# alanqrwang/nwhead

Hardware: AMD Instinct MI355X
Metric: query-predictions/sec (higher is better)
Workload: dtype f32; 1 GPU; K3 predict('full'): B=256 queries/step vs bank N=50000 d=512 C=200, bank sharded 1-way, 26 query batches coalesced per launch; B=256, N_support=50000, d=512, C=200, parallelism=support-shard x1

## Files before the change

### nwhead_amd/csrc/fused.hip

```cpp
#include <mutex>
#include <utility>
#include <vector>
#include "fused_impl.h"

namespace nw {

#define NW_EXTERN_FUSED_KIND(K) extern template int launch_fused_kind<K>(const FusedArgs&, const FusedPlan&);
NW_FOR_EACH_KIND(NW_EXTERN_FUSED_KIND)
#undef NW_EXTERN_FUSED_KIND

namespace {
struct TileTimer {
    bool on = false;
    std::vector<std::pair<hipEvent_t, hipEvent_t>> ev;
    std::vector<std::pair<hipEvent_t, hipEvent_t>> pool;
    std::mutex mu;
} g_tt;
}

int tile_timer_start(hipStream_t st) {
    if (!g_tt.on) return -1;
    std::lock_guard<std::mutex> lk(g_tt.mu);
    std::pair<hipEvent_t, hipEvent_t> p;
    if (!g_tt.pool.empty()) {
        p = g_tt.pool.back();
        g_tt.pool.pop_back();
    } else if (hipEventCreate(&p.first) != hipSuccess || hipEventCreate(&p.second) != hipSuccess) {
        return -1;
    }
    (void)hipEventRecord(p.first, st);
    g_tt.ev.push_back(p);
    return (int)g_tt.ev.size() - 1;
}
void tile_timer_stop(int slot, hipStream_t st) {
    if (slot < 0) return;
    std::lock_guard<std::mutex> lk(g_tt.mu);
    if (slot < (int)g_tt.ev.size()) (void)hipEventRecord(g_tt.ev[slot].second, st);
}
int tile_timer_enable(bool on) {
    std::lock_guard<std::mutex> lk(g_tt.mu);
    g_tt.on = on;
    return NW_OK;
}
int tile_timer_read(double* total_us, int64_t* launches) {
    std::lock_guard<std::mutex> lk(g_tt.mu);
    double tot = 0;
    for (auto& p : g_tt.ev) {
        float ms = 0.f;
        if (hipEventSynchronize(p.second) != hipSuccess || hipEventElapsedTime(&ms, p.first, p.second) != hipSuccess)
            return NW_ERR_LAUNCH;
        tot += (double)ms * 1e3;
        g_tt.pool.push_back(p);
    }
    if (total_us) *total_us = tot;
    if (launches) *launches = (int64_t)g_tt.ev.size();
    g_tt.ev.clear();
    return NW_OK;
}

namespace {
int device_cu_count() {
    static int n = [] {
        int dev = 0, v = 0;
        if (hipGetDevice(&dev) != hipSuccess) return 256;
        if (hipDeviceGetAttribute(&v, hipDeviceAttributeMultiprocessorCount, dev) != hipSuccess || v <= 0) return 256;
        return v;
    }();
    return n;
}
bool env_flag(int k) { return knob(k) == 1; }
}

inline size_t al256(size_t x) { return (x + 255) & ~(size_t)255; }

size_t fused_layout(int64_t B, int64_t n_stiles, int BS, char* base, FusedWs* ws, int64_t C) {
    size_t off = 0;
    auto take = [&](size_t bytes) {
        char* p = base ? base + off : nullptr;
        off += al256(bytes);
        return p;
    };
    FusedWs w;
    w.m = reinterpret_cast<float*>(take((size_t)n_stiles * B * 4));
    w.den = reinterpret_cast<float*>(take((size_t)n_stiles * B * 4));
    w.nrun = reinterpret_cast<int*>(take((size_t)n_stiles * 4));
    w.lab = reinterpret_cast<int*>(take((size_t)n_stiles * BS * 4));
    w.num = reinterpret_cast<float*>(take((size_t)n_stiles * BS * B * 4));
    w.runid = reinterpret_cast<int*>(take(((size_t)n_stiles * BS + 64) * 4));
    w.bnd = reinterpret_cast<int*>(take((size_t)n_stiles * 2 * 4));
    w.ctab = reinterpret_cast<int*>(take((size_t)C * (3 + 4) * 4));
    if (ws) *ws = w;
    return off;
}

namespace {

constexpr int MTHREADS = 512, MENT = 4, MTPT = 16;
template <bool PARTIAL, int MQ, int TMODE>
__global__ __launch_bounds__(MTHREADS) void nw_merge_runs_kernel(
    const float* __restrict__ ws_m, const float* __restrict__ ws_den, const int* __restrict__ ws_nrun,
    const int* __restrict__ ws_lab, const float* __restrict__ ws_num, float* __restrict__ out,
    float* __restrict__ lse, float* __restrict__ m_out, float* __restrict__ den_out,
    float* __restrict__ num_out, int B, int C, int n_stiles, int BS, const int* __restrict__ ctab) {
    constexpr bool TABLES = TMODE != 0;
    constexpr bool LTAB = TMODE == 1;
    constexpr int ML = MTHREADS / MQ;
    constexpr int MNS = MQ + 1;
    constexpr int NW = MTHREADS / 64;
    constexpr float LN2 = 0.693147180559945309417f;
    static_assert(MQ <= 32 && (MQ & (MQ - 1)) == 0, "a wave holds whole groups of MQ queries");
    extern __shared__ __attribute__((aligned(16))) char smem[];
    float* red = reinterpret_cast<float*>(smem);
    float* Ms = red + 2 * NW * MQ;
    float* inv_s = Ms + MQ;
    int* lds_tab = reinterpret_cast<int*>(inv_s + MQ);
    int* cnt = TMODE == 2 ? const_cast<int*>(ctab) : lds_tab;
    int* tlo = cnt + C;
    int* thi = tlo + C;
    int* ent = thi + C;
    float* res = reinterpret_cast<float*>(lds_tab + (size_t)C * (3 + MENT));
    const int tid = threadIdx.x, bq = tid & (MQ - 1), sl = tid / MQ, wave = tid >> 6;
    const int b0 = blockIdx.x * MQ;
    const int b = min(b0 + bq, B - 1);

    const bool in_regs = n_stiles <= ML * MTPT;
    float mr[MTPT], dr[MTPT];
    float M = -INFINITY;
    if (in_regs) {
#pragma unroll
        for (int u = 0; u < MTPT; ++u) {
            const int t = sl + u * ML;
            const bool ok = t < n_stiles;
            mr[u] = ok ? ws_m[(size_t)t * B + b] : -INFINITY;
            dr[u] = ok ? ws_den[(size_t)t * B + b] : 0.f;
        }
    }
    int tnr = 0, tl3[3] = {-1, -1, -1};
    const bool one_pass_tables = LTAB && n_stiles <= MTHREADS;
    if (one_pass_tables && tid < n_stiles) {
        tnr = ws_nrun[tid];
        const int* lt = ws_lab + (size_t)tid * BS;
        tl3[0] = lt[0];
        tl3[1] = lt[1];
        tl3[2] = lt[2];
    }
    if (LTAB) {
        for (int c = tid; c < C; c += MTHREADS) {
            cnt[c] = 0;
            tlo[c] = 0x7fffffff;
            thi[c] = -1;
        }
    }
    if (in_regs) {
#pragma unroll
        for (int u = 0; u < MTPT; ++u) M = fmaxf(M, mr[u]);
    } else {
        for (int t = sl; t < n_stiles; t += ML) M = fmaxf(M, ws_m[(size_t)t * B + b]);
    }
#pragma unroll
    for (int o = 32; o >= MQ; o >>= 1) M = fmaxf(M, __shfl_xor(M, o));
    if ((tid & 63) < MQ) red[wave * MQ + bq] = M;
    __syncthreads();
    if (LTAB) {
        auto add_tile = [&](int t, int nr, const int (&l3)[3]) {
            const int* lt = ws_lab + (size_t)t * BS;
            for (int r = 0; r < nr; ++r) {
                const int y = r < 3 ? l3[r] : lt[r];
                if (y < 0) continue;
                atomicMin(&tlo[y], t);
                atomicMax(&thi[y], t);
                const int slot = atomicAdd(&cnt[y], 1);
                if (slot < MENT) ent[y * MENT + slot] = t * BS + r;
            }
        };
        if (one_pass_tables) {
            if (tid < n_stiles) add_tile(tid, tnr, tl3);
        } else {
            for (int t = tid; t < n_stiles; t += MTHREADS) {
                const int* lt = ws_lab + (size_t)t * BS;
                const int l3[3] = {lt[0], lt[1], lt[2]};
                add_tile(t, ws_nrun[t], l3);
            }
        }
    }
    M = red[bq];
#pragma unroll
    for (int k = 1; k < NW; ++k) M = fmaxf(M, red[k * MQ + bq]);
    float den = 0.f;
    if (in_regs) {
#pragma unroll
        for (int u = 0; u < MTPT; ++u) den += dr[u] * __builtin_amdgcn_exp2f(mr[u] - M);
    } else {
        for (int t = sl; t < n_stiles; t += ML)
            den += ws_den[(size_t)t * B + b] * __builtin_amdgcn_exp2f(ws_m[(size_t)t * B + b] - M);
    }
#pragma unroll
    for (int o = 32; o >= MQ; o >>= 1) den += __shfl_xor(den, o);
    if ((tid & 63) < MQ) red[NW * MQ + wave * MQ + bq] = den;
    if (sl == 0) Ms[bq] = M;
    __syncthreads();
    if (LTAB) {
        for (int c = tid; c < C; c += MTHREADS) {
            const int n = cnt[c];
            if (n > 1 && n <= MENT) {
                int e[MENT];
#pragma unroll
                for (int k = 0; k < MENT; ++k) e[k] = k < n ? ent[c * MENT + k] : 0x7fffffff;
#pragma unroll
                for (int i = 1; i < MENT; ++i)
#pragma unroll
                    for (int j = MENT - 1; j >= i; --j)
                        if (e[j] < e[j - 1]) { const int x = e[j]; e[j] = e[j - 1]; e[j - 1] = x; }
#pragma unroll
                for (int k = 0; k < MENT; ++k)
                    if (k < n) ent[c * MENT + k] = e[k];
            }
        }
    }
    den = red[NW * MQ + bq];
#pragma unroll
    for (int k = 1; k < NW; ++k) den += red[NW * MQ + k * MQ + bq];
    if (sl == 0) inv_s[bq] = 1.f / den;
    const int nq = min(MQ, B - b0);
    if (sl == 0 && bq < nq) {
        if (PARTIAL) {
            m_out[b] = M * LN2;
            den_out[b] = den;
        } else if (lse) {
            lse[b] = M * LN2 + logf(den);
        }
    }
    __syncthreads();
    int P = 1;
    while (P < 64 && 2 * P * C * MQ <= MTHREADS) P <<= 1;
    for (int xx = tid; xx < C * MQ * P; xx += MTHREADS) {
        const int x = xx / P, sub = xx - x * P;
        const int c = x / MQ, q = x - c * MQ;
        const int bb = min(b0 + q, B - 1);
        const float Mq = Ms[q];
        float acc = 0.f;
        const int n = TABLES ? cnt[c] : MENT + 1;
        if (n <= MENT) {
            int e[MENT];
            float v[MENT], mt[MENT];
#pragma unroll
            for (int k = 0; k < MENT; ++k) e[k] = ent[c * MENT + (k < n ? k : 0)];
#pragma unroll
            for (int k = 0; k < MENT; ++k) {
                if (k < n) {
                    v[k] = ws_num[(size_t)e[k] * B + bb];
                    mt[k] = ws_m[(size_t)(e[k] / BS) * B + bb];
                }
            }
#pragma unroll
            for (int k = 0; k < MENT; ++k)
                if (k < n) acc += v[k] * __builtin_amdgcn_exp2f(mt[k] - Mq);
        } else {
            const int t0 = TABLES ? tlo[c] : 0, t1 = TABLES ? thi[c] : n_stiles - 1;
            for (int t = t0 + sub; t <= t1; t += P) {
                const int nr = ws_nrun[t];
                const float f = __builtin_amdgcn_exp2f(ws_m[(size_t)t * B + bb] - Mq);
                const int* lt = ws_lab + (size_t)t * BS;
                for (int r = 0; r < nr; ++r)
                    if (lt[r] == c) acc += ws_num[((size_t)t * BS + r) * B + bb] * f;
            }
        }
        if (P > 1) {
            if (n <= MENT && sub != 0) acc = 0.f;
            for (int o = P >> 1; o > 0; o >>= 1) acc += __shfl_xor(acc, o);
            if (sub != 0) continue;
        }
        if (LTAB && MQ > 1) {
            res[c * MNS + q] = acc;
        } else if (q < nq) {
            if (PARTIAL) num_out[(size_t)bb * C + c] = acc;
            else out[(size_t)bb * C + c] = logf(acc * inv_s[q] + NW_LOG_EPS);
        }
    }
    if (!LTAB || MQ == 1) return;
    __syncthreads();
    for (int x = tid; x < nq * C; x += MTHREADS) {
        const int qq = x / C, c = x - qq * C;
        if (PARTIAL) num_out[(size_t)(b0 + qq) * C + c] = res[c * MNS + qq];
        else out[(size_t)(b0 + qq) * C + c] = logf(res[c * MNS + qq] * inv_s[qq] + NW_LOG_EPS);
    }
}

__global__ __launch_bounds__(1024) void nw_class_tables_kernel(const int* __restrict__ ws_nrun, const int* __restrict__ ws_lab,
                                                                int n_stiles, int BS, int C, int* __restrict__ ctab) {
    int* cnt = ctab;
    int* tlo = cnt + C;
    int* thi = tlo + C;
    int* ent = thi + C;
    const int tid = threadIdx.x;
    for (int c = tid; c < C; c += 1024) {
        cnt[c] = 0;
        tlo[c] = 0x7fffffff;
        thi[c] = -1;
    }
    __threadfence();
    __syncthreads();
    for (int t = tid; t < n_stiles; t += 1024) {
        const int nr = ws_nrun[t];
        const int* lt = ws_lab + (size_t)t * BS;
        for (int r = 0; r < nr; ++r) {
            const int y = lt[r];
            if (y < 0) continue;
            atomicMin(&tlo[y], t);
            atomicMax(&thi[y], t);
            const int slot = atomicAdd(&cnt[y], 1);
            if (slot < MENT) ent[y * MENT + slot] = t * BS + r;
        }
    }
    __threadfence();
    __syncthreads();
    for (int c = tid; c < C; c += 1024) {
        const int n = cnt[c];
        if (n > 1 && n <= MENT) {
            int e[MENT];
#pragma unroll
            for (int k = 0; k < MENT; ++k) e[k] = k < n ? ent[c * MENT + k] : 0x7fffffff;
#pragma unroll
            for (int i = 1; i < MENT; ++i)
#pragma unroll
                for (int j = MENT - 1; j >= i; --j)
                    if (e[j] < e[j - 1]) { const int x = e[j]; e[j] = e[j - 1]; e[j - 1] = x; }
#pragma unroll
            for (int k = 0; k < MENT; ++k)
                if (k < n) ent[c * MENT + k] = e[k];
        }
    }
}

__global__ __launch_bounds__(64) void nw_run_tables_kernel(const int64_t* __restrict__ sy, int N, int C, int BS,
                                                           int* __restrict__ runid, int* __restrict__ nrun,
                                                           int* __restrict__ lab_out, int* __restrict__ bnd) {
    const int st = blockIdx.x, lane = threadIdx.x, s0 = st * BS;
    if (lane < 2) bnd[2 * st + lane] = BS;
    __syncthreads();
    int lab[3], flag[3];
#pragma unroll
    for (int u = 0; u < 3; ++u) {
        const int t = 3 * lane + u, j = s0 + t;
        int64_t y = -1;
        if (t < BS && j < N) y = sy[j];
        lab[u] = ((uint64_t)y < (uint64_t)C) ? (int)y : -1;
    }
    const int prev_last = __shfl_up(lab[2], 1);
    flag[0] = (lane == 0) || (lab[0] != prev_last);
    flag[1] = lab[1] != lab[0];
    flag[2] = lab[2] != lab[1];
    int incl = flag[0] + flag[1] + flag[2];
#pragma unroll
    for (int o = 1; o < 64; o <<= 1) {
        const int v = __shfl_up(incl, o);
        if (lane >= o) incl += v;
    }
    int id = incl - (flag[0] + flag[1] + flag[2]) - 1;
#pragma unroll
    for (int u = 0; u < 3; ++u) {
        const int t = 3 * lane + u;
        id += flag[u];
        if (t < BS) {
            runid[(size_t)s0 + t] = id;
            if (flag[u]) lab_out[(size_t)s0 + id] = lab[u];
            if (flag[u] && (id == 1 || id == 2)) bnd[2 * st + id - 1] = t;
            if (t == BS - 1) nrun[st] = id + 1;
        }
    }
}

int env_rs() {
    const int v = knob(KNOB_TILE_RS);
    return v == KNOB_UNSET ? 0 : v;
}

}

int query_area_of_workspace(void* workspace, size_t workspace_bytes, int64_t B, int64_t N, int64_t d, int64_t C, float** rows,
                            float** scale, float** norm2) {
    const size_t total = nw_fwd_workspace_bytes(B, N, d, C);
    if (!workspace || workspace_bytes < total) return NW_ERR_WORKSPACE;
    const size_t a = al256((size_t)B * (size_t)d * sizeof(float)), b = al256((size_t)B * sizeof(float));
    char* base = static_cast<char*>(workspace) + (total - a - 3 * b);
    *rows = reinterpret_cast<float*>(base);
    *scale = reinterpret_cast<float*>(base + a);
    *norm2 = reinterpret_cast<float*>(base + a + b);
    return NW_OK;
}

int launch_run_tables(const FusedWs& ws, const int64_t* sy, int N, int C, int n_stiles, int BS, hipStream_t st) {
    if (BS > 192) return NW_ERR_UNSUPPORTED;
    hipLaunchKernelGGL(nw_run_tables_kernel, dim3(n_stiles), dim3(64), 0, st, sy, N, C, BS, ws.runid, ws.nrun, ws.lab, ws.bnd);
    NW_CHECK_LAUNCH();
    return NW_OK;
}

constexpr int BANK_BS = 128;

size_t bank_tables_layout(int64_t n_stiles, char* base, FusedWs* ws) {
    size_t off = 0;
    auto take = [&](size_t bytes) {
        char* p = base ? base + off : nullptr;
        off += al256(bytes);
        return p;
    };
    int* nrun = reinterpret_cast<int*>(take((size_t)n_stiles * 4));
    int* lab = reinterpret_cast<int*>(take((size_t)n_stiles * BANK_BS * 4));
    int* runid = reinterpret_cast<int*>(take(((size_t)n_stiles * BANK_BS + 64) * 4));
    int* bnd = reinterpret_cast<int*>(take((size_t)n_stiles * 2 * 4));
    if (ws) {
        ws->nrun = nrun;
        ws->lab = lab;
        ws->runid = runid;
        ws->bnd = bnd;
    }
    return off;
}

bool bank_tables_take(const int64_t* sy, int N, int C, int n_stiles, int BS, FusedWs* ws) {
    (void)C;
    const FwdOpts& o = fwd_opts();
    if (!o.tables || BS != BANK_BS) return false;
    if (o.tables_sy != sy || o.tables_N != (int64_t)N) return false;
    if (o.tables_bytes < bank_tables_layout(n_stiles, nullptr, nullptr)) return false;
    bank_tables_layout(n_stiles, const_cast<char*>(o.tables), ws);
    return true;
}

int launch_merge_runs(const FusedWs& ws, float* out, float* lse, float* m, float* den, float* num,
                      int B, int C, int n_stiles, int BS, hipStream_t st) {
    auto lds_bytes = [&](int mq, bool tables) {
        return ((size_t)2 * (MTHREADS / 64) * mq + 2 * mq + (tables ? (size_t)C * (3 + MENT + mq + 1) : 0)) * sizeof(float);
    };
    const size_t cap = 150 * 1024;
    int mq = 1;
    const int force_mq = knob(KNOB_MERGE_MQ) == KNOB_UNSET ? 0 : knob(KNOB_MERGE_MQ);
    if (force_mq == 1 || force_mq == 16 || force_mq == 32) {
        mq = force_mq;
        if (lds_bytes(mq, true) > cap) mq = 1;
    } else if (B >= 512 && !env_flag(KNOB_MERGE_PER_QUERY)) {
        mq = n_stiles >= 128 ? 16 : 32;
        if (lds_bytes(mq, true) > cap) mq = 16;
        if (lds_bytes(mq, true) > cap) mq = 1;
    }
    const bool tables = lds_bytes(mq, true) <= cap;
    const size_t lds = lds_bytes(mq, tables);
    const int grid = (B + mq - 1) / mq;
#define NW_MERGE(P_, Q_, T_)                                                                                       \
    hipLaunchKernelGGL((nw_merge_runs_kernel<P_, Q_, T_>), dim3(grid), dim3(MTHREADS), lds, st, ws.m, ws.den, ws.nrun, \
                       ws.lab, ws.num, out, lse, m, den, num, B, C, n_stiles, BS, ws.ctab)
    if (!tables) {
        if (ws.ctab && !env_flag(KNOB_MERGE_NO_GLOBAL_TABLES)) {
            hipLaunchKernelGGL(nw_class_tables_kernel, dim3(1), dim3(1024), 0, st, ws.nrun, ws.lab, n_stiles, BS, C, ws.ctab);
            if (out) NW_MERGE(false, 1, 2); else NW_MERGE(true, 1, 2);
        } else {
            if (out) NW_MERGE(false, 1, 0); else NW_MERGE(true, 1, 0);
        }
    } else if (mq == 1) {
        if (out) NW_MERGE(false, 1, 1); else NW_MERGE(true, 1, 1);
    } else if (mq == 16) {
        if (out) NW_MERGE(false, 16, 1); else NW_MERGE(true, 16, 1);
    } else {
        if (out) NW_MERGE(false, 32, 1); else NW_MERGE(true, 32, 1);
    }
#undef NW_MERGE
    NW_CHECK_LAUNCH();
    return NW_OK;
}

int pick_rs(int64_t B, int64_t N, int64_t d, bool f16) {
    const int forced = env_rs();
    if (forced == 2 || forced == 4 || forced == 5 || forced == 6 || forced == 8 || forced == 10 || forced == 12)
        return forced;
    const int64_t nq = (B + BQ - 1) / BQ;
    if (forced == 0 && !f16 && d % BK == 0 && nq * ((N + 79) / 80) >= 480) return 5;
    if (forced == 0 && f16 && d % BK == 0 && nq * ((N + 127) / 128) >= 4 * 256) return 8;
    const int cand[] = {2, 4, 6, 8, 10, 12};
    const int ncand = f16 ? 5 : 6;
    double best = 1e30;
    int best_rs = 8;
    for (int ci = 0; ci < ncand; ++ci) {
        const int rs = cand[ci];
        const int64_t ns = (N + 16 * rs - 1) / (16 * rs);
        const int64_t nwg = nq * ns;
        const int64_t rounds = (nwg + 255) / 256;
        double cost = (double)rounds * (rs + 1.5);
        if (nwg >= 384) cost *= 0.85;
        if (cost < best - 1e-9) {
            best = cost;
            best_rs = rs;
        }
    }
    return best_rs;
}

bool half_form_shape_ok(int64_t d) {
    return d % 64 == 0 && d >= 192 && d <= (1 << 20);
}

namespace {
struct TileLds {
    size_t reg, dma;
    size_t p64, p64x2, p128;
};
template <int RS>
constexpr TileLds tile_lds() {
    if constexpr (RS > 5)
        return {FUSED_HDR + TileCfg<RS>::STAGE_BYTES, FUSED_HDR + DmaCfg<RS>::STAGE_BYTES, PCfg<RS, 1, false>::LDS_BYTES,
                PCfg<RS, 1, true>::LDS_BYTES, PCfg<RS, 2, false>::LDS_BYTES};
    else
        return {FUSED_HDR + TileCfg<RS>::STAGE_BYTES, FUSED_HDR + DmaCfg<RS>::STAGE_BYTES, 0, 0, 0};
}
TileLds tile_lds_of(int rs) {
    return rs == 2 ? tile_lds<2>() : rs == 4 ? tile_lds<4>() : rs == 5 ? tile_lds<5>() : rs == 6 ? tile_lds<6>()
         : rs == 8 ? tile_lds<8>() : rs == 10 ? tile_lds<10>() : tile_lds<12>();
}
}

FusedPlan plan_tiles(int64_t B, int64_t N, int64_t d, int form) {
    FusedPlan p = {};
    p.form = form;
    p.rs = form == FORM_HALF ? BANK_BS / 16 : pick_rs(B, N, d, form == FORM_SPLIT);
    p.BS = 16 * p.rs;
    const int64_t n_stiles = (N + p.BS - 1) / p.BS, n_qtiles = (B + BQ - 1) / BQ;
    const int64_t grid = (n_stiles + 7) / 8 * 8 * n_qtiles;
    if (grid > 0x7fffffff) p.status = NW_ERR_UNSUPPORTED;
    else p.n_stiles = (int)n_stiles, p.n_qtiles = (int)n_qtiles, p.grid = (int)grid;
    return p;
}

FusedPlan plan_fused(int64_t B, int64_t N, int64_t d, int64_t C, int form, int out, int k, bool norms, bool dot, int cus,
                     const FwdOpts& opts) {
    (void)C; (void)k;
    if (B < 0 || N < 0 || d < 0 || B >= (1 << 30) || N >= (1 << 30) || d >= (1 << 30)) {
        FusedPlan none = {};
        return none.status = NW_ERR_UNSUPPORTED, none;
    }
    FusedPlan p = plan_tiles(B, N, d, form);
    if (p.status != NW_OK) return p;
    auto refuse = [&p](int status) { p.status = status; return p; };
    if (cus <= 0) cus = device_cu_count();
    const TileLds lds = tile_lds_of(p.rs);
    const bool split = form == FORM_SPLIT;
    p.out = out;
    p.dma = (d % BK) == 0 && (uint64_t)(BQ + p.BS) * 2 * d * 4 < 0xffffffffull;
    if (form == FORM_HALF) {
        if (out != OUT_NONE || !half_form_shape_ok(d)) return refuse(NW_ERR_UNSUPPORTED);
        p.persistent = true;
    } else {
        if (!p.dma && (p.rs & 1)) return refuse(NW_ERR_UNSUPPORTED);
        p.persistent = split && out == OUT_NONE && p.rs > 5 && (p.rs == 8 || env_flag(KNOB_PERSISTENT_ANY_RS)) &&
                       p.grid >= 4 * (int64_t)cus && d >= 3 * BK && !env_flag(KNOB_NO_PERSISTENT);
    }
    p.run_tables = p.persistent;
    if (p.run_tables && p.BS > 192) return refuse(NW_ERR_UNSUPPORTED);
    if (split && (!p.dma || !norms)) return refuse(NW_ERR_INVALID_ARG);
    if (out == OUT_CAND && !split) return refuse(NW_ERR_INVALID_ARG);
    if (out == OUT_CAND && p.rs == 12) return refuse(NW_ERR_UNSUPPORTED);
    if (p.persistent) {
        p.mode = MODE_F16;
        p.split_queries = true;
        int wgs = cus & ~7;
        const int wg_cap = opts.persistent_wgs & ~7;
        if (wg_cap >= 8 && wg_cap < wgs) wgs = wg_cap;
        int variant = form == FORM_HALF ? 3 : knob(KNOB_PVAR);
        if (variant < 0 || variant > 3) {
            const double rows64 = 1.15 * ((B + 63) / 64 * 64);
            variant = (p.rs == 8 && (B + 255) / 256 * 256 <= rows64) ? 3 : ((B + 127) / 128 * 128 <= rows64) ? 2 : 1;
        }
        if (variant == 3 && p.rs != 8) variant = 2;
        if (variant == 2 && lds.p128 > 160 * 1024) variant = 0;
        if (variant == 1 && lds.p64x2 > 80 * 1024) variant = 0;
        p.variant = variant;
        p.workgroups = variant == 1 ? 2 * wgs : wgs;
        const int qg = (knob(KNOB_QG) >= 1 && knob(KNOB_QG) <= 64) ? knob(KNOB_QG) : 8;
        p.qgroup = variant != 3 ? qg : qg >= 2 ? qg / 2 : 1;
        p.lds_bytes = variant == 3 ? (size_t)P12::LDS_BYTES : variant == 2 ? lds.p128 : variant == 1 ? lds.p64x2 : lds.p64;
        return p;
    }
    if (split) {
        const int force_split = knob(KNOB_SPLIT_QUERIES) == KNOB_UNSET ? -1 : knob(KNOB_SPLIT_QUERIES);
        const bool raw_ok = force_split == 0 || (force_split < 0 && 2 * (int64_t)p.grid <= 3 * (int64_t)cus);
        p.split_queries = !raw_ok;
        p.mode = raw_ok ? MODE_F16Q : MODE_F16;
    } else {
        p.mode = !p.dma ? MODE_REG : (norms && !dot) ? MODE_DMA_SN : MODE_DMA;
    }
    p.lds_bytes = p.mode == MODE_REG ? lds.reg : lds.dma;
    return p;
}

size_t fused_workspace_bytes(int64_t B, int64_t N, int64_t d, int64_t C) {
    size_t need = 0;
    for (int form : {FORM_F32, FORM_SPLIT, FORM_HALF}) {
        if (form == FORM_HALF && !half_form_shape_ok(d)) continue;
        const int BS = plan_tiles(B, N, d, form).BS;
        const size_t n = fused_layout(B, (N + BS - 1) / BS, BS, nullptr, nullptr, C);
        need = n > need ? n : need;
    }
    return need;
}

bool fused_eligible(const float* q, const float* s, int64_t B, int64_t N, int64_t d, int64_t C) {
    const bool aligned = ((reinterpret_cast<uintptr_t>(q) | reinterpret_cast<uintptr_t>(s)) & 15) == 0;
    return N > 25 && d >= 4 && (d % 4) == 0 && aligned && B < (1 << 30) && N < (1 << 30) &&
           d < (1 << 30) && C < (1 << 30) && (8 + C) * 4 <= 160 * 1024;
}

int launch_fused(const FusedArgs& a, int form, int kind) {
    const int out = a.cand ? OUT_CAND : a.scores ? OUT_SCORES : OUT_NONE;
    const FusedPlan p = plan_fused(a.B, a.N, a.d, a.C, form, out, a.cand ? a.cand->k : 0, a.s_norm2 != nullptr,
                                   kind == NW_SCORE_DOT, 0, fwd_opts());
#define NW_KIND_CASE(K) case K: return launch_fused_kind<K>(a, p);
    switch (kind) {
        NW_FOR_EACH_KIND(NW_KIND_CASE)
        default: return NW_ERR_UNSUPPORTED;
    }
#undef NW_KIND_CASE
}

namespace {
struct KnnWs {
    CandOut cand;
    int64_t n_stiles;
    int kcp;
};
bool knn_shape_ok(int64_t B, int64_t N, int64_t d, int64_t k) {
    return B >= 0 && N > 25 && d >= BK && d % BK == 0 && k >= 1 && k <= 32 && k <= N && B < (1 << 30) && N < (1 << 30) &&
           d <= (1 << 20);
}
size_t knn_layout(int64_t B, int64_t N, int64_t d, int64_t k, int BS, char* base, KnnWs* out) {
    KnnWs w;
    w.n_stiles = (N + BS - 1) / BS;
    w.kcp = cand_slots((int)k, BS);
    size_t off = 0;
    auto take = [&](size_t bytes) {
        char* p = base ? base + off : nullptr;
        off += al256(bytes);
        return p;
    };
    const size_t slots = (size_t)B * (size_t)w.n_stiles * (size_t)w.kcp;
    w.cand.key = reinterpret_cast<unsigned*>(take(slots * 4));
    w.cand.row = reinterpret_cast<int*>(take(slots * 4));
    w.cand.q_rows = reinterpret_cast<float*>(take((size_t)B * (size_t)d * 4));
    w.cand.q_scale = reinterpret_cast<float*>(take((size_t)B * 4));
    w.cand.q_norm2 = reinterpret_cast<float*>(take((size_t)B * 4));
    w.cand.k = (int)k;
    if (out) *out = w;
    return off;
}
}

size_t knn_workspace_bytes(int64_t B, int64_t N, int64_t d, int64_t k) {
    if (!knn_shape_ok(B, N, d, k) || B == 0) return 0;
    if (pick_rs(B, N, d, true) > 10) return 0;
    size_t need = knn_layout(B, N, d, k, 16 * pick_rs(B, N, d, true), nullptr, nullptr);
    const int64_t nq = (B + BQ - 1) / BQ;
    for (int64_t qt = 1; qt <= nq && qt < 1024; ++qt) {
        const int64_t Bq = qt * BQ < B ? qt * BQ : B;
        for (int64_t n = 17; n <= N && qt * ((n + 127) / 128) < 1024; n += 16) {
            const int64_t nn = n > 26 ? n : 26;
            if (nn > N || k > nn) continue;
            const size_t x = knn_layout(Bq, nn, d, k, 16 * pick_rs(Bq, nn, d, true), nullptr, nullptr);
            need = x > need ? x : need;
        }
    }
    return need;
}

int launch_knn(const float* q, const float* s_split, const float* s_scale, const float* s_norm2, int64_t* idx, float* vals,
               void* workspace, size_t workspace_bytes, int64_t B, int64_t N, int64_t d, int64_t k, int kind, const float* ls,
               hipStream_t st) {
    if (!knn_shape_ok(B, N, d, k)) return NW_ERR_UNSUPPORTED;
    if (B == 0) return NW_OK;
    KnnWs w;
    const size_t need = knn_layout(B, N, d, k, plan_tiles(B, N, d, FORM_SPLIT).BS, static_cast<char*>(workspace), &w);
    if (!workspace || workspace_bytes < need) return NW_ERR_WORKSPACE;
    if (w.n_stiles * w.kcp >= (1ll << 31)) return NW_ERR_UNSUPPORTED;
    FusedArgs a = {};
    a.q = q, a.s = s_split, a.s_norm2 = s_norm2, a.s_scale = s_scale, a.ls = ls;
    a.B = (int)B, a.N = (int)N, a.d = (int)d, a.C = 1, a.st = st, a.cand = &w.cand;
    const int rc = launch_fused(a, FORM_SPLIT, kind);
    if (rc != NW_OK) return rc;
    return launch_topk_candidates(w.cand.key, w.cand.row, idx, vals, B, w.n_stiles * w.kcp, k, st);
}

}

extern "C" size_t nw_bank_tables_bytes(int64_t N) {
    if (N <= 0 || N > 0x7fffffffLL) return 0;
    return nw::bank_tables_layout((N + nw::BANK_BS - 1) / nw::BANK_BS, nullptr, nullptr);
}

extern "C" int nw_bank_tables_build(const int64_t* sy, int64_t N, int64_t C, void* tables, size_t tables_bytes,
                                    void* stream) {
    using namespace nw;
    if (N < 0 || C < 0 || N > 0x7fffffffLL || C > 0x7fffffffLL) return NW_ERR_INVALID_ARG;
    if (N == 0) return NW_OK;
    if (!sy || !tables || (reinterpret_cast<uintptr_t>(tables) & 15)) return NW_ERR_INVALID_ARG;
    const int64_t n_stiles = (N + BANK_BS - 1) / BANK_BS;
    FusedWs ws;
    if (tables_bytes < bank_tables_layout(n_stiles, static_cast<char*>(tables), &ws)) return NW_ERR_WORKSPACE;
    return launch_run_tables(ws, sy, (int)N, (int)C, (int)n_stiles, BANK_BS, static_cast<hipStream_t>(stream));
}
```

Baseline: 7.781 million query-predictions/s.

## Merge two query groups per merge block and batch fast-path class gathers

When the merge kernel runs with 16 queries per block, it can now launch 1024-thread blocks covering two query groups. This shares the per-block class-table build across twice as many queries and halves the grid. The class-entry path is split into a batched pass that issues several items' gathers before doing the exp/accumulate, to hide global load latency. It also packs tile/row indices to avoid a division, and walks the final output loop incrementally instead of dividing each iteration. In exchange it adds register pressure and more LDS per block, and the packing assumes BS is at most 256.

```diff
diff --git a/nwhead_amd/csrc/fused.hip b/nwhead_amd/csrc/fused.hip
--- a/nwhead_amd/csrc/fused.hip
+++ b/nwhead_amd/csrc/fused.hip
@@ -96,31 +96,38 @@
 namespace {
 
 constexpr int MTHREADS = 512, MENT = 4, MTPT = 16;
-template <bool PARTIAL, int MQ, int TMODE>
-__global__ __launch_bounds__(MTHREADS) void nw_merge_runs_kernel(
+__device__ __forceinline__ int ment_pack(int t, int r) { return (t << 8) | r; }
+template <bool PARTIAL, int MQ, int TMODE, int G>
+__global__ __launch_bounds__(MTHREADS * G) void nw_merge_runs_kernel(
     const float* __restrict__ ws_m, const float* __restrict__ ws_den, const int* __restrict__ ws_nrun,
     const int* __restrict__ ws_lab, const float* __restrict__ ws_num, float* __restrict__ out,
     float* __restrict__ lse, float* __restrict__ m_out, float* __restrict__ den_out,
     float* __restrict__ num_out, int B, int C, int n_stiles, int BS, const int* __restrict__ ctab) {
     constexpr bool TABLES = TMODE != 0;
     constexpr bool LTAB = TMODE == 1;
+    constexpr int NT = MTHREADS * G;
+    constexpr int QW = MQ * G;
     constexpr int ML = MTHREADS / MQ;
-    constexpr int MNS = MQ + 1;
-    constexpr int NW = MTHREADS / 64;
+    constexpr int MNS = QW + 1;
+    constexpr int NW = NT / 64;
+    constexpr int MITEMS = G == 2 ? 7 : MQ == 1 ? 2 : 4;
     constexpr float LN2 = 0.693147180559945309417f;
     static_assert(MQ <= 32 && (MQ & (MQ - 1)) == 0, "a wave holds whole groups of MQ queries");
+    static_assert(G == 1 || (G == 2 && QW <= 32), "two groups: one more tile-lane bit comes from the wave number");
     extern __shared__ __attribute__((aligned(16))) char smem[];
     float* red = reinterpret_cast<float*>(smem);
-    float* Ms = red + 2 * NW * MQ;
-    float* inv_s = Ms + MQ;
-    int* lds_tab = reinterpret_cast<int*>(inv_s + MQ);
+    float* Ms = red + 2 * NW * QW;
+    float* inv_s = Ms + QW;
+    int* lds_tab = reinterpret_cast<int*>(inv_s + QW);
     int* cnt = TMODE == 2 ? const_cast<int*>(ctab) : lds_tab;
     int* tlo = cnt + C;
     int* thi = tlo + C;
     int* ent = thi + C;
     float* res = reinterpret_cast<float*>(lds_tab + (size_t)C * (3 + MENT));
-    const int tid = threadIdx.x, bq = tid & (MQ - 1), sl = tid / MQ, wave = tid >> 6;
-    const int b0 = blockIdx.x * MQ;
+    const int tid = threadIdx.x, wave = tid >> 6;
+    const int bq = tid & (QW - 1);
+    const int sl = G == 1 ? tid / MQ : (wave >> 1) * (64 / MQ) + 2 * ((tid & 63) / QW) + (wave & 1);
+    const int b0 = blockIdx.x * QW;
     const int b = min(b0 + bq, B - 1);
 
     const bool in_regs = n_stiles <= ML * MTPT;
@@ -136,7 +143,7 @@
         }
     }
     int tnr = 0, tl3[3] = {-1, -1, -1};
-    const bool one_pass_tables = LTAB && n_stiles <= MTHREADS;
+    const bool one_pass_tables = LTAB && n_stiles <= NT;
     if (one_pass_tables && tid < n_stiles) {
         tnr = ws_nrun[tid];
         const int* lt = ws_lab + (size_t)tid * BS;
@@ -145,7 +152,7 @@
         tl3[2] = lt[2];
     }
     if (LTAB) {
-        for (int c = tid; c < C; c += MTHREADS) {
+        for (int c = tid; c < C; c += NT) {
             cnt[c] = 0;
             tlo[c] = 0x7fffffff;
             thi[c] = -1;
@@ -158,8 +165,8 @@
         for (int t = sl; t < n_stiles; t += ML) M = fmaxf(M, ws_m[(size_t)t * B + b]);
     }
 #pragma unroll
-    for (int o = 32; o >= MQ; o >>= 1) M = fmaxf(M, __shfl_xor(M, o));
-    if ((tid & 63) < MQ) red[wave * MQ + bq] = M;
+    for (int o = 32; o >= QW; o >>= 1) M = fmaxf(M, __shfl_xor(M, o));
+    if ((tid & 63) < QW) red[wave * QW + bq] = M;
     __syncthreads();
     if (LTAB) {
         auto add_tile = [&](int t, int nr, const int (&l3)[3]) {
@@ -170,13 +177,13 @@
                 atomicMin(&tlo[y], t);
                 atomicMax(&thi[y], t);
                 const int slot = atomicAdd(&cnt[y], 1);
-                if (slot < MENT) ent[y * MENT + slot] = t * BS + r;
+                if (slot < MENT) ent[y * MENT + slot] = ment_pack(t, r);
             }
         };
         if (one_pass_tables) {
             if (tid < n_stiles) add_tile(tid, tnr, tl3);
         } else {
-            for (int t = tid; t < n_stiles; t += MTHREADS) {
+            for (int t = tid; t < n_stiles; t += NT) {
                 const int* lt = ws_lab + (size_t)t * BS;
                 const int l3[3] = {lt[0], lt[1], lt[2]};
                 add_tile(t, ws_nrun[t], l3);
@@ -185,7 +192,7 @@
     }
     M = red[bq];
 #pragma unroll
-    for (int k = 1; k < NW; ++k) M = fmaxf(M, red[k * MQ + bq]);
+    for (int k = 1; k < NW; ++k) M = fmaxf(M, red[k * QW + bq]);
     float den = 0.f;
     if (in_regs) {
 #pragma unroll
@@ -195,12 +202,12 @@
             den += ws_den[(size_t)t * B + b] * __builtin_amdgcn_exp2f(ws_m[(size_t)t * B + b] - M);
     }
 #pragma unroll
-    for (int o = 32; o >= MQ; o >>= 1) den += __shfl_xor(den, o);
-    if ((tid & 63) < MQ) red[NW * MQ + wave * MQ + bq] = den;
+    for (int o = 32; o >= QW; o >>= 1) den += __shfl_xor(den, o);
+    if ((tid & 63) < QW) red[NW * QW + wave * QW + bq] = den;
     if (sl == 0) Ms[bq] = M;
     __syncthreads();
     if (LTAB) {
-        for (int c = tid; c < C; c += MTHREADS) {
+        for (int c = tid; c < C; c += NT) {
             const int n = cnt[c];
             if (n > 1 && n <= MENT) {
                 int e[MENT];
@@ -217,11 +224,18 @@
             }
         }
     }
-    den = red[NW * MQ + bq];
-#pragma unroll
-    for (int k = 1; k < NW; ++k) den += red[NW * MQ + k * MQ + bq];
+    const float* dred = red + NW * QW;
+    if (G == 1) {
+        den = dred[bq];
+#pragma unroll
+        for (int k = 1; k < NW; ++k) den += dred[k * QW + bq];
+    } else {
+        den = dred[bq] + dred[QW + bq];
+#pragma unroll
+        for (int k = 1; k < NW / 2; ++k) den += dred[2 * k * QW + bq] + dred[(2 * k + 1) * QW + bq];
+    }
     if (sl == 0) inv_s[bq] = 1.f / den;
-    const int nq = min(MQ, B - b0);
+    const int nq = min(QW, B - b0);
     if (sl == 0 && bq < nq) {
         if (PARTIAL) {
             m_out[b] = M * LN2;
@@ -231,58 +245,91 @@
         }
     }
     __syncthreads();
-    int P = 1;
-    while (P < 64 && 2 * P * C * MQ <= MTHREADS) P <<= 1;
-    for (int xx = tid; xx < C * MQ * P; xx += MTHREADS) {
-        const int x = xx / P, sub = xx - x * P;
-        const int c = x / MQ, q = x - c * MQ;
+    int P = 1, lgP = 0;
+    while (P < 64 && 2 * P * C * MQ <= MTHREADS) { P <<= 1; ++lgP; }
+    const int n_items = P == 1 ? C * QW : NT;
+    auto item = [&](int xx, int& c, int& q, int& sub) {
+        if (P == 1) {
+            c = xx / QW, q = xx - c * QW, sub = 0;
+            return xx < n_items;
+        }
+        const int grp = xx / MTHREADS, xg = xx - grp * MTHREADS, x = xg >> lgP;
+        c = x / MQ, q = grp * MQ + (x - c * MQ), sub = xg - (x << lgP);
+        return xg < C * MQ * P;
+    };
+    auto emit = [&](int c, int q, float acc) {
+        if (LTAB && MQ > 1) {
+            res[c * MNS + q] = acc;
+        } else if (q < nq) {
+            const int bb = b0 + q;
+            if (PARTIAL) num_out[(size_t)bb * C + c] = acc;
+            else out[(size_t)bb * C + c] = logf(acc * inv_s[q] + NW_LOG_EPS);
+        }
+    };
+    if (TABLES) {
+        for (int base = tid; base < n_items; base += NT * MITEMS) {
+            float v[MITEMS][MENT], mt[MITEMS][MENT];
+            auto fast_item = [&](int i, int& c, int& q) {
+                int sub;
+                const bool ok = base + i * NT < n_items && item(base + i * NT, c, q, sub) && sub == 0;
+                const int n = ok ? cnt[c] : MENT + 1;
+                if (n <= MENT) return n;
+                c = 0, q = 0;
+                return -1;
+            };
+#pragma unroll
+            for (int i = 0; i < MITEMS; ++i) {
+                int c, q;
+                const int n = fast_item(i, c, q);
+                const int bb = min(b0 + q, B - 1), cc = n > 0 ? c : 0;
+#pragma unroll
+                for (int k = 0; k < MENT; ++k) {
+                    const int ek = ent[cc * MENT + (k < n ? k : 0)], e = n > 0 ? ek : 0;
+                    const unsigned t = (unsigned)e >> 8, row = t * BS + (e & 255);
+                    v[i][k] = ws_num[(size_t)row * (unsigned)B + bb];
+                    mt[i][k] = ws_m[(size_t)t * (unsigned)B + bb];
+                }
+            }
+#pragma unroll
+            for (int i = 0; i < MITEMS; ++i) {
+                int c, q;
+                const int n = fast_item(i, c, q);
+                const float Mq = Ms[q];
+                float acc = 0.f;
+#pragma unroll
+                for (int k = 0; k < MENT; ++k)
+                    if (k < n) acc += v[i][k] * __builtin_amdgcn_exp2f(mt[i][k] - Mq);
+                if (n >= 0) emit(c, q, acc);
+            }
+        }
+    }
+    for (int xx = tid; xx < n_items; xx += NT) {
+        int c, q, sub;
+        if (!item(xx, c, q, sub)) continue;
+        if (TABLES && cnt[c] <= MENT) continue;
         const int bb = min(b0 + q, B - 1);
         const float Mq = Ms[q];
         float acc = 0.f;
-        const int n = TABLES ? cnt[c] : MENT + 1;
-        if (n <= MENT) {
-            int e[MENT];
-            float v[MENT], mt[MENT];
-#pragma unroll
-            for (int k = 0; k < MENT; ++k) e[k] = ent[c * MENT + (k < n ? k : 0)];
-#pragma unroll
-            for (int k = 0; k < MENT; ++k) {
-                if (k < n) {
-                    v[k] = ws_num[(size_t)e[k] * B + bb];
-                    mt[k] = ws_m[(size_t)(e[k] / BS) * B + bb];
-                }
-            }
-#pragma unroll
-            for (int k = 0; k < MENT; ++k)
-                if (k < n) acc += v[k] * __builtin_amdgcn_exp2f(mt[k] - Mq);
-        } else {
-            const int t0 = TABLES ? tlo[c] : 0, t1 = TABLES ? thi[c] : n_stiles - 1;
-            for (int t = t0 + sub; t <= t1; t += P) {
-                const int nr = ws_nrun[t];
-                const float f = __builtin_amdgcn_exp2f(ws_m[(size_t)t * B + bb] - Mq);
-                const int* lt = ws_lab + (size_t)t * BS;
-                for (int r = 0; r < nr; ++r)
-                    if (lt[r] == c) acc += ws_num[((size_t)t * BS + r) * B + bb] * f;
-            }
-        }
-        if (P > 1) {
-            if (n <= MENT && sub != 0) acc = 0.f;
-            for (int o = P >> 1; o > 0; o >>= 1) acc += __shfl_xor(acc, o);
-            if (sub != 0) continue;
-        }
-        if (LTAB && MQ > 1) {
-            res[c * MNS + q] = acc;
-        } else if (q < nq) {
-            if (PARTIAL) num_out[(size_t)bb * C + c] = acc;
-            else out[(size_t)bb * C + c] = logf(acc * inv_s[q] + NW_LOG_EPS);
-        }
+        const int t0 = TABLES ? tlo[c] : 0, t1 = TABLES ? thi[c] : n_stiles - 1;
+        for (int t = t0 + sub; t <= t1; t += P) {
+            const int nr = ws_nrun[t];
+            const float f = __builtin_amdgcn_exp2f(ws_m[(size_t)t * B + bb] - Mq);
+            const int* lt = ws_lab + (size_t)t * BS;
+            for (int r = 0; r < nr; ++r)
+                if (lt[r] == c) acc += ws_num[((size_t)t * BS + r) * B + bb] * f;
+        }
+        for (int o = P >> 1; o > 0; o >>= 1) acc += __shfl_xor(acc, o);
+        if (sub == 0) emit(c, q, acc);
     }
     if (!LTAB || MQ == 1) return;
     __syncthreads();
-    for (int x = tid; x < nq * C; x += MTHREADS) {
-        const int qq = x / C, c = x - qq * C;
+    const int dq = NT / C, dc = NT - dq * C;
+    int qq = tid / C, c = tid - qq * C;
+    for (int x = tid; x < nq * C; x += NT) {
         if (PARTIAL) num_out[(size_t)(b0 + qq) * C + c] = res[c * MNS + qq];
         else out[(size_t)(b0 + qq) * C + c] = logf(res[c * MNS + qq] * inv_s[qq] + NW_LOG_EPS);
+        qq += dq, c += dc;
+        if (c >= C) c -= C, ++qq;
     }
 }
 
@@ -309,7 +356,7 @@
             atomicMin(&tlo[y], t);
             atomicMax(&thi[y], t);
             const int slot = atomicAdd(&cnt[y], 1);
-            if (slot < MENT) ent[y * MENT + slot] = t * BS + r;
+            if (slot < MENT) ent[y * MENT + slot] = ment_pack(t, r);
         }
     }
     __threadfence();
@@ -445,24 +492,30 @@
         if (lds_bytes(mq, true) > cap) mq = 1;
     }
     const bool tables = lds_bytes(mq, true) <= cap;
-    const size_t lds = lds_bytes(mq, tables);
-    const int grid = (B + mq - 1) / mq;
-#define NW_MERGE(P_, Q_, T_)                                                                                       \
-    hipLaunchKernelGGL((nw_merge_runs_kernel<P_, Q_, T_>), dim3(grid), dim3(MTHREADS), lds, st, ws.m, ws.den, ws.nrun, \
-                       ws.lab, ws.num, out, lse, m, den, num, B, C, n_stiles, BS, ws.ctab)
+    auto lds_bytes_g = [&](int g) {
+        return ((size_t)2 * (MTHREADS * g / 64) * mq * g + 2 * mq * g + (tables ? (size_t)C * (3 + MENT + mq * g + 1) : 0)) * sizeof(float);
+    };
+    const int groups = mq == 16 && lds_bytes_g(2) <= cap ? 2 : 1;
+    const size_t lds = lds_bytes_g(groups);
+    const int grid = (B + mq * groups - 1) / (mq * groups);
+#define NW_MERGE(P_, Q_, T_, G_)                                                                                   \
+    hipLaunchKernelGGL((nw_merge_runs_kernel<P_, Q_, T_, G_>), dim3(grid), dim3(MTHREADS * G_), lds, st, ws.m, ws.den, \
+                       ws.nrun, ws.lab, ws.num, out, lse, m, den, num, B, C, n_stiles, BS, ws.ctab)
     if (!tables) {
         if (ws.ctab && !env_flag(KNOB_MERGE_NO_GLOBAL_TABLES)) {
             hipLaunchKernelGGL(nw_class_tables_kernel, dim3(1), dim3(1024), 0, st, ws.nrun, ws.lab, n_stiles, BS, C, ws.ctab);
-            if (out) NW_MERGE(false, 1, 2); else NW_MERGE(true, 1, 2);
+            if (out) NW_MERGE(false, 1, 2, 1); else NW_MERGE(true, 1, 2, 1);
         } else {
-            if (out) NW_MERGE(false, 1, 0); else NW_MERGE(true, 1, 0);
+            if (out) NW_MERGE(false, 1, 0, 1); else NW_MERGE(true, 1, 0, 1);
         }
     } else if (mq == 1) {
-        if (out) NW_MERGE(false, 1, 1); else NW_MERGE(true, 1, 1);
+        if (out) NW_MERGE(false, 1, 1, 1); else NW_MERGE(true, 1, 1, 1);
+    } else if (mq == 16 && groups == 2) {
+        if (out) NW_MERGE(false, 16, 1, 2); else NW_MERGE(true, 16, 1, 2);
     } else if (mq == 16) {
-        if (out) NW_MERGE(false, 16, 1); else NW_MERGE(true, 16, 1);
+        if (out) NW_MERGE(false, 16, 1, 1); else NW_MERGE(true, 16, 1, 1);
     } else {
-        if (out) NW_MERGE(false, 32, 1); else NW_MERGE(true, 32, 1);
+        if (out) NW_MERGE(false, 32, 1, 1); else NW_MERGE(true, 32, 1, 1);
     }
 #undef NW_MERGE
     NW_CHECK_LAUNCH();
```

After: 7.820 million query-predictions/s, median of 6. About the same (+0.5%).
